# boqian-li/GarmentDreamer

Hardware: AMD Instinct MI355X
Metric: SDS iters/sec (rasterize+UNet+bwd), 100k Gaussians ×8 views @512², 1/2/4/8 GPU (higher is better)
Workload: dtype bf16

## Files before the change

garmentdreamer_amd/csrc/nn_conv3x3.hip:

```cpp
#include <hip/hip_runtime.h>
#include <stdlib.h>
#include <stdint.h>
#include <stdio.h>

#include <mutex>
#include <vector>

#include "../../include/gd_nn.h"
#include "nn_device.h"
#include "nn_host.h"

#ifndef GD_CONV_ABLATE
#define GD_CONV_ABLATE 0
#endif

namespace {

using namespace gdnn;

#ifndef GD_PATCH_EPI
#define GD_PATCH_EPI 0
#endif
typedef __attribute__((ext_vector_type(4))) float f32x4;

// ... 241 lines not shown

__device__ __forceinline__ float silu_fast(float z) { return z * __builtin_amdgcn_rcpf(1.0f + __expf(-z)); }

__device__ __forceinline__ float row16_sum(float v)
{
    v += __builtin_bit_cast(float, __builtin_amdgcn_update_dpp(0, __builtin_bit_cast(int, v), 0xB1, 0xf, 0xf, false));
    v += __builtin_bit_cast(float, __builtin_amdgcn_update_dpp(0, __builtin_bit_cast(int, v), 0x4E, 0xf, 0xf, false));
    v += __builtin_bit_cast(float, __builtin_amdgcn_update_dpp(0, __builtin_bit_cast(int, v), 0x141, 0xf, 0xf, false));
    v += __builtin_bit_cast(float, __builtin_amdgcn_update_dpp(0, __builtin_bit_cast(int, v), 0x140, 0xf, 0xf, false));
    return v;
}

__device__ __forceinline__ void stat_accumulate(float2& st, uint2 o)
{
    const float r0 = __uint_as_float(o.x << 16), r1 = __uint_as_float(o.x & 0xffff0000u);
    const float r2 = __uint_as_float(o.y << 16), r3 = __uint_as_float(o.y & 0xffff0000u);
    st.x += (r0 + r1) + (r2 + r3);
    st.y += fmaf(r0, r0, fmaf(r1, r1, fmaf(r2, r2, r3 * r3)));
}

__device__ __forceinline__ void patch_col(int fn, int& rr, int& fx)
{
    if (fn < 4) { rr = 0; fx = fn; }
    else if (fn < 12) { rr = 1; fx = fn - 4; }
    else if (fn < 16) { rr = 0; fx = fn - 8; }
    else if (fn < 20) { rr = 1; fx = fn - 8; }
    else if (fn < 28) { rr = 0; fx = fn - 12; }
    else { rr = 1; fx = fn - 16; }
}

constexpr int kTrRow = 80;
constexpr int kTrWave = 64 * kTrRow;

template <int BN, int WN, int FA, int FB>
__device__ __forceinline__ void patch_epilogue(f32x16 (&acc)[FA][FB], char* tr, int nimg, int tyi, int txi, int n0, int wc,
                                               int wp, int lane, int H, int W, int Cout, const uint16_t* __restrict__ bias,
                                               int bias_img_stride, const uint16_t* __restrict__ residual,
                                               uint16_t* __restrict__ out, float* __restrict__ stat_part, int tpi,
                                               int tiles_x)
{
    const int fk = lane >> 5, fn = lane & 31;
    int rr, fx;
    patch_col(fn, rr, fx);
    bool ok[FB];
    size_t opix[FB];
#pragma unroll
    for (int b = 0; b < FB; b++) {
        const int oy = tyi * 16 + 4 * wp + 2 * b + rr, ox = txi * 16 + fx;
        ok[b] = oy < H && ox < W;
        opix[b] = ((size_t)nimg * H + oy) * W + ox;
    }
    const uint16_t* bias_n = bias ? bias + (size_t)nimg * bias_img_stride : nullptr;
    const int stat_rows = tpi * 8;
    const int stat_row = (tyi * tiles_x + txi) * 8 + wp * 2 + ((lane >> 4) & 1);
    const bool wide = GD_PATCH_EPI != 2 && tr != nullptr && (Cout & 7) == 0;
#pragma unroll
    for (int a = 0; a < FA; a++) {
#pragma unroll
        for (int q = 0; q < 4; q++) {
            const int co = n0 + wc * (BN / WN) + a * 32 + 8 * q + 4 * fk;
            const bool cok = co < Cout;
            float bv[4] = {0.f, 0.f, 0.f, 0.f};
            if (bias_n && cok) {
                const uint2 bb = *(const uint2*)(bias_n + co);
                bv[0] = bf2f((uint16_t)(bb.x & 0xffff)); bv[1] = bf2f((uint16_t)(bb.x >> 16));
                bv[2] = bf2f((uint16_t)(bb.y & 0xffff)); bv[3] = bf2f((uint16_t)(bb.y >> 16));
            }
            float2 st = make_float2(0.f, 0.f);
#pragma unroll
            for (int b = 0; b < FB; b++) {
                if (!ok[b] || !cok) continue;
                float v[4];
#pragma unroll
                for (int e = 0; e < 4; e++) v[e] = acc[a][b][4 * q + e] + bv[e];
                if (residual) {
                    const uint2 rv = *(const uint2*)(residual + opix[b] * Cout + co);
                    v[0] += bf2f((uint16_t)(rv.x & 0xffff)); v[1] += bf2f((uint16_t)(rv.x >> 16));
                    v[2] += bf2f((uint16_t)(rv.y & 0xffff)); v[3] += bf2f((uint16_t)(rv.y >> 16));
                }
                uint2 o;
                o.x = pack_bf16(v[0], v[1]);
                o.y = pack_bf16(v[2], v[3]);
                if (wide) *(uint2*)(tr + (b * 32 + fn) * kTrRow + 16 * q + 8 * fk) = o;
                else if (GD_PATCH_EPI != 1 || H < 0) *(uint2*)(out + opix[b] * Cout + co) = o;
                if (stat_part) stat_accumulate(st, o);
            }
            if (stat_part) {
                const float sx = row16_sum(st.x), sy = row16_sum(st.y);
                if ((lane & 15) == 0 && cok)
                    *(float2*)(stat_part + (((size_t)nimg * (Cout >> 2) + (co >> 2)) * stat_rows + stat_row) * 2) =
                        make_float2(sx, sy);
            }
        }
        if (wide) {
            __builtin_amdgcn_wave_barrier();
#pragma unroll
            for (int i = 0; i < FB * 2; i++) {
                const int pr = (lane >> 2) + 16 * i, ch = lane & 3;
                int rr2, fx2;
                patch_col(pr & 31, rr2, fx2);
                const int oy = tyi * 16 + 4 * wp + 2 * (pr >> 5) + rr2, ox = txi * 16 + fx2;
                const int co8 = n0 + wc * (BN / WN) + a * 32 + 8 * ch;
                if (oy < H && ox < W && co8 < Cout) {
                    const uint4 v = *(const uint4*)(tr + pr * kTrRow + ch * 16);
                    if (GD_PATCH_EPI != 1 || H < 0) *(uint4*)(out + (((size_t)nimg * H + oy) * W + ox) * Cout + co8) = v;
                }
            }
            __builtin_amdgcn_wave_barrier();
        }
    }
}

template <int BN, int WN, int WM, bool GN>
__global__ __launch_bounds__(64 * WN * WM) void conv3x3_gn_patch_kernel(
    const uint16_t* __restrict__ in, const uint16_t* __restrict__ wt, const uint16_t* __restrict__ bias,
    int bias_img_stride, const uint16_t* __restrict__ residual, uint16_t* __restrict__ out, int Nimg, int H, int W,
    int Cin, int Cout, const float* __restrict__ mean_rstd, const uint16_t* __restrict__ gamma,
    const uint16_t* __restrict__ beta, int G, int apply_silu, int tiles_n, int tiles_x, int tiles_y, int nwg,
    float* __restrict__ stat_part)
{
    constexpr int BM = 256;
    constexpr int THREADS = 64 * WN * WM;
    constexpr int NB = BN * 8 / THREADS;
    constexpr int NA = (kPatchPix * 8 + THREADS - 1) / THREADS;
    constexpr int FA = BN / WN / 32, FB = BM / WM / 32;
    static_assert(FB == 2 && THREADS % 8 == 0, "wave pixel block = 4 patch rows x 16");
    constexpr int kAStage = (kPatchPix + 4) * BK * 2;
    constexpr int kBStage = BN * BK * 2;
    extern __shared__ __attribute__((aligned(16))) char smem[];
    char* sA = smem;
    char* sB = smem + 2 * kAStage;

    const int tid = threadIdx.x, lane = tid & 63;
    const int wave = __builtin_amdgcn_readfirstlane(tid >> 6);
    int bid = blockIdx.x;
    if ((nwg & 7) == 0) bid = (bid & 7) * (nwg >> 3) + (bid >> 3);
    const int tn = bid % tiles_n, tm = bid / tiles_n;
    const int tpi = tiles_x * tiles_y;
    const int nimg = tm / tpi, trem = tm - nimg * tpi;
// ... 133 lines not shown
                    if (tap == 0) loadA(c + 1);
                    else if (tap == 1) storeA((c + 1) & 1, c + 1);
                } else if (tap == 0) {
                    issueA((c + 1) & 1, c + 1);
                }
            }
            const char* pb = sB + bufB * kBStage;
            const int tapoff = (tap / 3) * kPatch + (tap % 3);
            uint32_t p_rd[FB], p_sw[FB];
#pragma unroll
            for (int b = 0; b < FB; b++) {
                const int p = p_base[b] + tapoff;
                p_rd[b] = (uint32_t)p * 128u;
                p_sw[b] = (uint32_t)((p >> 1) & 7);
            }
#pragma unroll
            for (int kk = 0; kk < 4; kk++) {
                bf16x8_t wf[FA], pf[FB];
#pragma unroll
                for (int a = 0; a < FA; a++) wf[a] = *(const bf16x8_t*)(pb + (w_rd[a] ^ (uint32_t)(kk << 5)));
#pragma unroll
                for (int b = 0; b < FB; b++)
                    pf[b] = *(const bf16x8_t*)(pa + p_rd[b] + ((((uint32_t)(2 * kk + fk)) ^ p_sw[b]) << 4));
#pragma unroll
                for (int a = 0; a < FA; a++)
#pragma unroll
                    for (int b = 0; b < FB; b++)
                        acc[a][b] = __builtin_amdgcn_mfma_f32_32x32x16_bf16(wf[a], pf[b], acc[a][b], 0, 0, 0);
            }
        }
    }

    if (GD_PATCH_EPI != 2) __syncthreads();
    patch_epilogue<BN, WN, FA, FB>(acc, sA + ((kc - 1) & 1) * kAStage + wave * kTrWave, nimg, tyi, txi, n0, wc, wp, lane, H, W,
                                   Cout, bias, bias_img_stride, residual, out, stat_part, tpi, tiles_x);
}

template <int BN, int WN, int WM, bool GN>
__global__ __launch_bounds__(64 * WN * WM) void conv3x3_patch_stream_kernel(
    const uint16_t* __restrict__ in, const uint16_t* __restrict__ wt, const uint16_t* __restrict__ bias,
    int bias_img_stride, const uint16_t* __restrict__ residual, uint16_t* __restrict__ out, int Nimg, int H, int W,
    int Cin, int Cout, const float* __restrict__ mean_rstd, const uint16_t* __restrict__ gamma,
    const uint16_t* __restrict__ beta, int G, int apply_silu, int tiles_n, int tiles_x, int tiles_y, int nwg,
    float* __restrict__ stat_part)
{
    constexpr int BM = 256;
    constexpr int THREADS = 64 * WN * WM;
    constexpr int NB = BN * 8 / THREADS;
    constexpr int NA = (kPatchPix * 8 + THREADS - 1) / THREADS;
    constexpr int FA = BN / WN / 32, FB = BM / WM / 32;
    static_assert(FB == 2 && THREADS % 8 == 0, "wave pixel block = 4 patch rows x 16");
    constexpr int kAStage = (kPatchPix + 4) * BK * 2;
    constexpr int kBStage = BN * BK * 2;
    extern __shared__ __attribute__((aligned(16))) char smem[];
    char* sA = smem;
    char* sB = smem + 2 * kAStage;

    const int tid = threadIdx.x, lane = tid & 63;
    const int wave = __builtin_amdgcn_readfirstlane(tid >> 6);
    const int tpi = tiles_x * tiles_y;
    const bool remap = (nwg & 7) == 0 && (GN || (gridDim.x & 7) == 0);
    struct Tile { int nimg, tyi, txi, n0; };
    auto decode = [&](int vb) {
        int bid = vb;
        if (remap) bid = (vb & 7) * (nwg >> 3) + (vb >> 3);
        const int tn = bid % tiles_n, tm = bid / tiles_n;
        Tile t;
        t.nimg = tm / tpi;
// ... 162 lines not shown
                        if (tap == 0) loadA(nc);
                        else if (tap == 1) storeA(st, nc);
                    } else if (tap == 0) {
                        issueA(st, nc);
                    }
                }
                const char* pb = sB + bufB * kBStage;
                const int tapoff = (tap / 3) * kPatch + (tap % 3);
                uint32_t p_rd[FB], p_sw[FB];
#pragma unroll
                for (int b = 0; b < FB; b++) {
                    const int p = p_base[b] + tapoff;
                    p_rd[b] = (uint32_t)p * 128u;
                    p_sw[b] = (uint32_t)((p >> 1) & 7);
                }
#pragma unroll
                for (int kk = 0; kk < 4; kk++) {
                    bf16x8_t wf[FA], pf[FB];
#pragma unroll
                    for (int a = 0; a < FA; a++) wf[a] = *(const bf16x8_t*)(pb + (w_rd[a] ^ (uint32_t)(kk << 5)));
#pragma unroll
                    for (int b = 0; b < FB; b++)
                        pf[b] = *(const bf16x8_t*)(pa + p_rd[b] + ((((uint32_t)(2 * kk + fk)) ^ p_sw[b]) << 4));
#pragma unroll
                    for (int a = 0; a < FA; a++)
#pragma unroll
                        for (int b = 0; b < FB; b++)
                            acc[a][b] = __builtin_amdgcn_mfma_f32_32x32x16_bf16(wf[a], pf[b], acc[a][b], 0, 0, 0);
                }
            }
        }

        if (GD_PATCH_EPI != 2) __syncthreads();
        patch_epilogue<BN, WN, FA, FB>(acc, sA + ((ga - 1) & 1) * kAStage + wave * kTrWave, cur.nimg, cur.tyi, cur.txi, cur.n0,
                                       wc, wp, lane, H, W, Cout, bias, bias_img_stride, residual, out, stat_part, tpi,
                                       tiles_x);
        if (!has_next) break;
        cur = nxt;
        vb = vnext;
#pragma unroll
        for (int a = 0; a < FA; a++)
#pragma unroll
            for (int b = 0; b < FB; b++)
#pragma unroll
                for (int k = 0; k < 16; k++) acc[a][b][k] = 0.f;
    }
}

#include "nn_conv_wino.h"
#include "nn_conv_wide.h"
#include "nn_conv_first_dgrad.h"
#ifdef GD_NN_EXPERIMENTAL_STREAM
#include "nn_conv_stream.h"
#endif
#ifdef GD_NN_EXPERIMENTAL_REGW
#include "nn_conv_regw.h"
#endif

template <int BM_T>
__global__ __launch_bounds__(256) void conv_splitk_reduce_kernel(const float* __restrict__ partial, int S, int nwg,
                                                                 int tiles_n, int64_t M, int Cout, int HWg, int Wg, int Hout,
                                                                 int Wout, int osy, int osx, int ooy, int oox,
                                                                 const uint16_t* __restrict__ bias, int bias_img_stride,
                                                                 const uint16_t* __restrict__ residual,
                                                                 uint16_t* __restrict__ out)
{
    constexpr int kQuads = 128 * BM_T / 4, kBlocks = kQuads / 256;
    const int tile = blockIdx.x / kBlocks;
    const int r = ((blockIdx.x % kBlocks) << 8) | threadIdx.x;
    const int lane = r & 63, q = (r >> 6) & 3, a = (r >> 8) & 1, b = (r >> 9) & 1, wave = r >> 10;
    const int tn = tile % tiles_n, tm = tile / tiles_n;
    const int64_t m = (int64_t)tm * BM_T + (wave >> 1) * 64 + b * 32 + (lane & 31);
    const int co = tn * 128 + (wave & 1) * 64 + a * 32 + 8 * q + 4 * (lane >> 5);
    if (m >= M || co >= Cout) return;
    float4 v = make_float4(0.f, 0.f, 0.f, 0.f);
    const float4* p = (const float4*)partial + (size_t)tile * kQuads + r;
    for (int sidx = 0; sidx < S; sidx++) {
        const float4 t = p[(size_t)sidx * nwg * kQuads];
        v.x += t.x; v.y += t.y; v.z += t.z; v.w += t.w;
    }
    const size_t nimg = (size_t)(m / HWg);
    const int rem = (int)(m - (int64_t)nimg * HWg);
    const int ga = rem / Wg, gb = rem - ga * Wg;
    const size_t o = ((nimg * Hout + (size_t)(ga * osy + ooy)) * Wout + (size_t)(gb * osx + oox)) * Cout + co;
    if (bias) {
        const uint2 bb = *(const uint2*)(bias + nimg * (size_t)bias_img_stride + co);
        v.x += bf2f((uint16_t)(bb.x & 0xffff)); v.y += bf2f((uint16_t)(bb.x >> 16));
        v.z += bf2f((uint16_t)(bb.y & 0xffff)); v.w += bf2f((uint16_t)(bb.y >> 16));
    }
    if (residual) {
        const uint2 rr = *(const uint2*)(residual + o);
        v.x += bf2f((uint16_t)(rr.x & 0xffff)); v.y += bf2f((uint16_t)(rr.x >> 16));
        v.z += bf2f((uint16_t)(rr.y & 0xffff)); v.w += bf2f((uint16_t)(rr.y >> 16));
    }
    uint2 ov;
    ov.x = pack_bf16(v.x, v.y);
    ov.y = pack_bf16(v.z, v.w);
    *(uint2*)(out + o) = ov;
}

template <int CIN>
__global__ __launch_bounds__(256) void conv3x3_first_kernel(const uint16_t* __restrict__ in,
                                                            const uint16_t* __restrict__ wt,
                                                            const uint16_t* __restrict__ bias,
                                                            uint16_t* __restrict__ out, int Nimg, int H, int W, int Cout)
{
    constexpr int PX = 4;
    extern __shared__ __attribute__((aligned(16))) float s_w[];
    const int K = 9 * CIN;
    for (int i = threadIdx.x; i < K * Cout; i += 256) {
        const int k = i / Cout, co = i - k * Cout;
        s_w[i] = bf2f(wt[(size_t)co * K + k]);
    }
    __syncthreads();
    const int octs = Cout >> 3;
    const int oct = threadIdx.x % octs, grp = threadIdx.x / octs;
    const int gpb = 256 / octs;
    const int gx = (W + PX - 1) / PX;
    const int64_t total = (int64_t)Nimg * H * gx;
    if (grp >= gpb) return;
    for (int64_t g = (int64_t)blockIdx.x * gpb + grp; g < total; g += (int64_t)gridDim.x * gpb) {
    const int n = (int)((uint32_t)g / (uint32_t)(H * gx));
    const int rem = (int)((uint32_t)g - (uint32_t)n * (uint32_t)(H * gx));
    const int y = rem / gx, x0 = (rem - y * gx) * PX;

    float acc[PX][8];
    {
// ... 238 lines not shown
        if (b) g_cprof.pool.push_back(b);
    }
    void close_s1(int64_t M, int Cin, int Cout, bool residual)
    {
        close(2.0 * (double)M * Cout * 9.0 * Cin,
              2.0 * ((double)M * Cin + 9.0 * Cin * Cout + (double)M * Cout + (residual ? (double)M * Cout : 0.0)));
    }
};

struct TiledArgs {
    void* stream;
    const void* x;
    const float* mean_rstd;
    const void *gamma, *beta;
    int groups, silu;
    const void *w, *bias;
    int bias_img_stride;
    const void* residual;
    void* y;
    int N, H, W, Cin, Cout;
    float* stat_part;
};
constexpr int kCuLds = 160 * 1024;
static bool gn_table_fits(int lds, int Cin) { return lds + gn_table_bytes(Cin) <= kCuLds; }
template <auto Kern>
int launch_tiled(const TiledArgs& a, int lds, int tile_w, int bn, bool persistent)
{
    const int dev = current_device();
    if (dev < 0) return dev;
    if (a.mean_rstd) {
        if (!gn_table_fits(lds, a.Cin)) return fail(GD_NN_ERR_INVALID_ARG, "GroupNorm scale / shift table of Cin channels does not fit the LDS");
        lds += gn_table_bytes(a.Cin);
    }
    if (const int r = reserve_lds<Kern>(dev, a.mean_rstd ? kCuLds : lds)) return r;
    hipStream_t s = (hipStream_t)a.stream;
    const int tiles_x = (a.W + tile_w - 1) / tile_w, tiles_y = (a.H + 15) / 16, tiles_n = (a.Cout + bn - 1) / bn;
    const int nwg = a.N * tiles_x * tiles_y * tiles_n;
    int grid = nwg;
    if (persistent && nwg > num_cus(dev)) grid = (nwg & 7) == 0 ? (num_cus(dev) & ~7) : num_cus(dev);
    ProfScope prof(s);
    hipLaunchKernelGGL(Kern, dim3(grid), dim3(512), lds, s, (const uint16_t*)a.x, (const uint16_t*)a.w,
                       (const uint16_t*)a.bias, a.bias_img_stride, (const uint16_t*)a.residual, (uint16_t*)a.y, a.N, a.H,
                       a.W, a.Cin, a.Cout, a.mean_rstd, (const uint16_t*)a.gamma, (const uint16_t*)a.beta, a.groups, a.silu,
                       tiles_n, tiles_x, tiles_y, nwg, a.stat_part);
    prof.close_s1((int64_t)a.N * a.H * a.W, a.Cin, a.Cout, a.residual != nullptr);
    return launch_status();
}

}

extern "C" {

const char* gd_nn_conv_last_error(void) { return g_err; }

static int pick_split(int64_t tiles, int steps, int target = 420)
{
    int s = (int)((target + tiles / 2) / tiles);
    const int cap = steps * 2 / 15 < 24 ? steps * 2 / 15 : 24;
    if (s > cap) s = cap;
    return s < 2 ? 1 : s;
}

static size_t split_ws_bytes(int split, int64_t M, int Cout)
{
    return (size_t)split * (size_t)((M + 255) / 256 * 2) * (size_t)((Cout + 127) / 128) * 16384u * sizeof(float);
}
// ... 718 lines not shown
```

garmentdreamer_amd/csrc/nn_conv_wide.h:

```cpp
#pragma once
#include "nn_device.h"

constexpr int kWideCK = 32;
constexpr int kWidePW = 34, kWidePix = 18 * kWidePW;
constexpr int kWidePStage = 2560 * 16;
constexpr int kWideWStage = 3 * 128 * kWideCK * 2;
constexpr int kWideLds = 2 * kWidePStage + 2 * kWideWStage;

__global__ __launch_bounds__(256) void conv3x3_wide_weights_kernel(const uint16_t* __restrict__ w, uint16_t* __restrict__ u,
                                                                   int Cout, int Cin)
{
    const int kc = Cin / kWideCK;
    const int tiles_n = (Cout + 127) / 128;
    const size_t total = (size_t)tiles_n * 3 * kc * 1536;
    for (size_t i = (size_t)blockIdx.x * blockDim.x + threadIdx.x; i < total; i += (size_t)gridDim.x * blockDim.x) {
        const int q = (int)(i % 1536);
        const size_t sl = i / 1536;
        const int c = (int)(sl % kc);
        const int ky = (int)((sl / kc) % 3);
        const int tn = (int)(sl / kc / 3);
        const int pc = q & 3, row = (q >> 2) & 127, kx = q >> 9;
        const int co = tn * 128 + row;
        const int ci0 = c * kWideCK + ((pc ^ ((row >> 2) & 3)) << 3);
        uint4 v = make_uint4(0u, 0u, 0u, 0u);
// ... 140 lines not shown
                    issueP((c + 1) & 1, c + 1);
                }
            }
            const char* pw = sW + bufW * kWideWStage;
#pragma unroll 1
            for (int kx = 0; kx < 3; kx++) {
                uint32_t p_rd[4], p_sw[4];
#pragma unroll
                for (int b = 0; b < 4; b++) {
                    const int p = p_base[b] + ky * kWidePW + kx;
                    p_rd[b] = (uint32_t)p * 64u;
                    p_sw[b] = (uint32_t)((p >> 2) & 3);
                }
#pragma unroll
                for (int kk = 0; kk < 2; kk++) {
                    const uint32_t ch = (uint32_t)(kk * 2 + fk);
                    bf16x8_t wf[2], pf[4];
#pragma unroll
                    for (int a = 0; a < 2; a++)
                        wf[a] = *(const bf16x8_t*)(pw + kx * (128 * 64) + a_rd[a] + ((ch ^ a_key) << 4));
#pragma unroll
                    for (int b = 0; b < 4; b++) pf[b] = *(const bf16x8_t*)(pa + p_rd[b] + ((ch ^ p_sw[b]) << 4));
#pragma unroll
                    for (int a = 0; a < 2; a++)
#pragma unroll
                        for (int b = 0; b < 4; b++)
                            acc[a][b] = __builtin_amdgcn_mfma_f32_32x32x16_bf16(wf[a], pf[b], acc[a][b], 0, 0, 0);
                }
            }
        }
    }

    __syncthreads();
    char* tr = smem + wave * kTrWave;
    const uint16_t* bias_n = bias ? bias + (size_t)nimg * bias_img_stride : nullptr;
    const int stat_rows = ((H + 15) / 16) * ((W + 15) / 16) * 8;
#pragma unroll
    for (int bh = 0; bh < 2; bh++) {
        bool ok[2];
        size_t opix[2];
#pragma unroll
        for (int j = 0; j < 2; j++) {
            const int oy = tyi * 16 + 4 * wr + 2 * j + rr, ox = txi * 32 + 16 * bh + fx;
            ok[j] = oy < H && ox < W;
            opix[j] = ((size_t)nimg * H + oy) * W + ox;
        }
        const int t16x = (W + 15) / 16, cx = 2 * txi + bh;
        const int stat_row = (tyi * t16x + cx) * 8 + wr * 2 + ((lane >> 4) & 1);
#pragma unroll
        for (int a = 0; a < 2; a++) {
#pragma unroll
            for (int q = 0; q < 4; q++) {
                const int co = n0 + wc * 64 + a * 32 + 8 * q + 4 * fk;
                const bool cok = co < Cout;
                float bv[4] = {0.f, 0.f, 0.f, 0.f};
                if (bias_n && cok) {
                    const uint2 bb = *(const uint2*)(bias_n + co);
                    bv[0] = bf2f((uint16_t)(bb.x & 0xffff)); bv[1] = bf2f((uint16_t)(bb.x >> 16));
                    bv[2] = bf2f((uint16_t)(bb.y & 0xffff)); bv[3] = bf2f((uint16_t)(bb.y >> 16));
                }
                float2 st = make_float2(0.f, 0.f);
#pragma unroll
                for (int j = 0; j < 2; j++) {
                    if (!ok[j] || !cok) continue;
                    const int b = 2 * bh + j;
                    float v[4];
#pragma unroll
                    for (int e = 0; e < 4; e++) v[e] = acc[a][b][4 * q + e] + bv[e];
                    if (residual) {
                        const uint2 rv = *(const uint2*)(residual + opix[j] * Cout + co);
                        v[0] += bf2f((uint16_t)(rv.x & 0xffff)); v[1] += bf2f((uint16_t)(rv.x >> 16));
                        v[2] += bf2f((uint16_t)(rv.y & 0xffff)); v[3] += bf2f((uint16_t)(rv.y >> 16));
                    }
                    uint2 o;
                    o.x = pack_bf16(v[0], v[1]);
                    o.y = pack_bf16(v[2], v[3]);
                    *(uint2*)(tr + (j * 32 + fn) * kTrRow + 16 * q + 8 * fk) = o;
                    if (stat_part) stat_accumulate(st, o);
                }
                if (stat_part) {
                    const float sx = row16_sum(st.x), sy = row16_sum(st.y);
                    if ((lane & 15) == 0 && cok && cx < t16x)
                        *(float2*)(stat_part + (((size_t)nimg * (Cout >> 2) + (co >> 2)) * stat_rows + stat_row) * 2) =
                            make_float2(sx, sy);
                }
            }
            __builtin_amdgcn_wave_barrier();
#pragma unroll
            for (int i = 0; i < 4; i++) {
                const int pr = (lane >> 2) + 16 * i, ch = lane & 3;
                int rr2, fx2;
                patch_col(pr & 31, rr2, fx2);
                const int oy = tyi * 16 + 4 * wr + 2 * (pr >> 5) + rr2, ox = txi * 32 + 16 * bh + fx2;
                const int co8 = n0 + wc * 64 + a * 32 + 8 * ch;
                if (oy < H && ox < W && co8 < Cout) {
                    const uint4 v = *(const uint4*)(tr + pr * kTrRow + ch * 16);
                    *(uint4*)(out + (((size_t)nimg * H + oy) * W + ox) * Cout + co8) = v;
                }
            }
            __builtin_amdgcn_wave_barrier();
        }
    }
}
```

garmentdreamer_amd/csrc/nn_conv_wino.h:

```cpp
#pragma once
#include "nn_device.h"

#ifndef GD_WINO_ABLATE
#define GD_WINO_ABLATE 0
#endif

constexpr int kWinoCK = 32;
constexpr int kWinoVStage = 4 * 18 * 8 * kWinoCK * 2;
constexpr int kWinoWStage = 4 * 128 * kWinoCK * 2;
constexpr int kWinoPBytes = 21 * 1024;
constexpr int kWinoLds = 2 * kWinoVStage + 2 * kWinoWStage + kWinoPBytes;

__device__ __forceinline__ uint16_t f2bf_finite(float f)
{
    uint32_t u = __float_as_uint(f);
    u += 0x7fffu + ((u >> 16) & 1u);
    return (uint16_t)(u >> 16);
}

__global__ __launch_bounds__(256) void conv3x3_wino_weights_kernel(const uint16_t* __restrict__ w,
                                                                   uint16_t* __restrict__ u, int Cout, int Cin)
{
    const int kc = Cin / kWinoCK;
    const int tiles_n = (Cout + 127) / 128;
// ... 214 lines not shown
#pragma unroll
                        for (int a = 0; a < 2; a++)
#pragma unroll
                            for (int b = 0; b < 2; b++) acc[p][a][b][0] += (float)wf[a][0] * (float)vf[b][1];
                    } else {
#pragma unroll
                        for (int a = 0; a < 2; a++)
#pragma unroll
                            for (int b = 0; b < 2; b++)
                                acc[p][a][b] = __builtin_amdgcn_mfma_f32_32x32x16_bf16(wf[a], vf[b], acc[p][a][b], 0, 0, 0);
                    }
                }
            }
        }
    }

    __syncthreads();
    if (GD_WINO_ABLATE != 5) {
        char* mine = smem + wave * 16384;
#pragma unroll
        for (int a = 0; a < 2; a++)
#pragma unroll
            for (int b = 0; b < 2; b++) {
#pragma unroll
                for (int q = 0; q < 4; q++) {
                    f32x4 sd;
#pragma unroll
                    for (int e = 0; e < 4; e++) sd[e] = pp ? acc[0][a][b][4 * q + e] : acc[1][a][b][4 * q + e];
                    *(f32x4*)(mine + ((a * 2 + b) * 4 + q) * 1024 + lane * 16) = sd;
                }
            }
    }
    __syncthreads();
    {
        const char* theirs = smem + (wave ^ 1) * 16384;
#pragma unroll
        for (int a = 0; a < 2; a++)
#pragma unroll
            for (int b = 0; b < 2; b++)
#pragma unroll
                for (int q = 0; q < 4; q++) {
                    const f32x4 rv = GD_WINO_ABLATE == 5 ? f32x4{0.f, 1.f, 2.f, 3.f}
                                                         : *(const f32x4*)(theirs + ((a * 2 + b) * 4 + q) * 1024 + lane * 16);
#pragma unroll
                    for (int e = 0; e < 4; e++) {
                        const float sm = acc[0][a][b][4 * q + e] + acc[1][a][b][4 * q + e];
                        acc[0][a][b][4 * q + e] = pp ? rv[e] - sm : sm + rv[e];
                    }
                }
    }
    __syncthreads();

    char* tr = smem + wave * kTrWave;
    bool ok[2];
    size_t opix[2];
#pragma unroll
    for (int b = 0; b < 2; b++) {
        const int oy = tyi * 16 + wq * 8 + b * 4 + (fn >> 3), ox = txi * 16 + 2 * (fn & 7) + pp;
        ok[b] = oy < H && ox < W;
        opix[b] = ((size_t)nimg * H + oy) * W + ox;
    }
    const uint16_t* bias_n = bias ? bias + (size_t)nimg * bias_img_stride : nullptr;
    const int stat_rows = tpi * 8;
    const int stat_row = (tyi * tiles_x + txi) * 8 + (pp * 2 + wq) * 2 + ((lane >> 4) & 1);
    const bool wide = (Cout & 7) == 0;
#pragma unroll
    for (int a = 0; a < 2; a++) {
#pragma unroll
        for (int q = 0; q < 4; q++) {
            const int co = n0 + wc * 64 + a * 32 + 8 * q + 4 * fk;
            const bool cok = co < Cout;
            float bv[4] = {0.f, 0.f, 0.f, 0.f};
            if (bias_n && cok) {
                const uint2 bb = *(const uint2*)(bias_n + co);
                bv[0] = bf2f((uint16_t)(bb.x & 0xffff)); bv[1] = bf2f((uint16_t)(bb.x >> 16));
                bv[2] = bf2f((uint16_t)(bb.y & 0xffff)); bv[3] = bf2f((uint16_t)(bb.y >> 16));
            }
            float2 st = make_float2(0.f, 0.f);
#pragma unroll
            for (int b = 0; b < 2; b++) {
                if (!ok[b] || !cok) continue;
                float v[4];
#pragma unroll
                for (int e = 0; e < 4; e++) v[e] = acc[0][a][b][4 * q + e] + bv[e];
                if (residual) {
                    const uint2 rv = *(const uint2*)(residual + opix[b] * Cout + co);
                    v[0] += bf2f((uint16_t)(rv.x & 0xffff)); v[1] += bf2f((uint16_t)(rv.x >> 16));
                    v[2] += bf2f((uint16_t)(rv.y & 0xffff)); v[3] += bf2f((uint16_t)(rv.y >> 16));
                }
                uint2 o;
                o.x = pack_bf16(v[0], v[1]);
                o.y = pack_bf16(v[2], v[3]);
                if (wide) *(uint2*)(tr + (b * 32 + fn) * kTrRow + 16 * q + 8 * fk) = o;
                else *(uint2*)(out + opix[b] * Cout + co) = o;
                if (stat_part) stat_accumulate(st, o);
            }
            if (stat_part) {
                const float sx = row16_sum(st.x), sy = row16_sum(st.y);
                if ((lane & 15) == 0 && cok)
                    *(float2*)(stat_part + (((size_t)nimg * (Cout >> 2) + (co >> 2)) * stat_rows + stat_row) * 2) =
                        make_float2(sx, sy);
            }
        }
        if (wide) {
            __builtin_amdgcn_wave_barrier();
#pragma unroll
            for (int i = 0; i < 4; i++) {
                const int pr = (lane >> 2) + 16 * i, ch = lane & 3;
                const int oy = tyi * 16 + wq * 8 + (pr >> 5) * 4 + ((pr & 31) >> 3), ox = txi * 16 + 2 * (pr & 7) + pp;
                const int co8 = n0 + wc * 64 + a * 32 + 8 * ch;
                if (oy < H && ox < W && co8 < Cout) {
                    const uint4 v = *(const uint4*)(tr + pr * kTrRow + ch * 16);
                    if (GD_WINO_ABLATE != 6 || H < 0) *(uint4*)(out + (((size_t)nimg * H + oy) * W + ox) * Cout + co8) = v;
                }
            }
            __builtin_amdgcn_wave_barrier();
        }
    }
}
```

garmentdreamer_amd/csrc/nn_device.h:

```cpp
#pragma once
#include <hip/hip_runtime.h>
#include <stdint.h>

namespace gdnn {

typedef __attribute__((ext_vector_type(8))) short bf16x8_t;
typedef __attribute__((ext_vector_type(16))) float f32x16;
typedef __attribute__((ext_vector_type(2))) float f32x2_t;
typedef __attribute__((ext_vector_type(2))) __bf16 bf16x2_t;
using f2 = f32x2_t;
using bf2_t = bf16x2_t;

struct alignas(16) bf16x8 {
    uint16_t v[8];
};
struct alignas(16) u32x4 { uint32_t w[4]; };

__device__ __forceinline__ float bf2f(uint16_t b) { return __uint_as_float(((uint32_t)b) << 16); }
__device__ __forceinline__ uint16_t f2bf(float f)
{
    uint32_t u = __float_as_uint(f);
    if ((u & 0x7fffffffu) > 0x7f800000u) return (uint16_t)((u >> 16) | 0x40);
    u += 0x7fffu + ((u >> 16) & 1u);
    return (uint16_t)(u >> 16);
}

__device__ __forceinline__ float lo16(uint32_t u) { return __uint_as_float(u << 16); }
__device__ __forceinline__ float hi16(uint32_t u) { return __uint_as_float(u & 0xffff0000u); }
__device__ __forceinline__ f2 unpack2(uint32_t w) { return f2{lo16(w), hi16(w)}; }
__device__ __forceinline__ uint32_t pack2(f2 v) { return __builtin_bit_cast(uint32_t, __builtin_convertvector(v, bf2_t)); }
__device__ __forceinline__ uint32_t pack_bf16(float lo, float hi) { return pack2(f2{lo, hi}); }
__device__ __forceinline__ f2 round_bf16(f2 v) { return unpack2(pack2(v)); }

__device__ __forceinline__ __amdgpu_buffer_rsrc_t buffer_rsrc(const void* p, uint32_t bytes)
{
    return __builtin_amdgcn_make_buffer_rsrc((void*)p, 0, (int)bytes, 0x00020000);
}

constexpr uint32_t kOOB = 0x80000000u;

__device__ __forceinline__ void bload_lds16(__amdgpu_buffer_rsrc_t rsrc, uint32_t voff, uint32_t soff, char* lds_wave_base)
{
    __builtin_amdgcn_raw_ptr_buffer_load_lds(rsrc, (__attribute__((address_space(3))) void*)lds_wave_base, 16, voff, soff,
                                             0, 0);
}

__device__ __forceinline__ int swz(int row, int j)
{
    return (row >> 1) * 256 + (((((row & 1) << 3) | j) ^ ((row >> 1) & 15)) << 4);
}

constexpr int gn_table_bytes(int Cin) { return 8 * Cin; }

__device__ __forceinline__ void gn_scale_shift(float gm, float bt, float mean, float rstd, float& sc, float& sh)
{
    sc = gm * rstd;
    sh = __builtin_fmaf(-mean, sc, bt);
}

__device__ __forceinline__ void gn_table_fill(uint32_t tab_off, int tid, int nthreads, int Cin, int G, int nimg,
                                              const float* __restrict__ mean_rstd, const uint16_t* __restrict__ gamma,
                                              const uint16_t* __restrict__ beta)
{
    const int cg = Cin / G;
    for (int ch = tid; ch < Cin; ch += nthreads) {
        const float2 mr = *(const float2*)(mean_rstd + ((size_t)nimg * G + ch / cg) * 2);
        float sc, sh;
        gn_scale_shift(bf2f(gamma[ch]), bf2f(beta[ch]), mr.x, mr.y, sc, sh);
        const uint32_t a = tab_off + (uint32_t)(((ch >> 3) * 16 + (ch & 7)) * 4);
        asm volatile("ds_write_b32 %0, %1\n\tds_write_b32 %0, %2 offset:32" ::"v"(a), "v"(sc), "v"(sh) : "memory");
    }
}

__device__ __forceinline__ void gn_table_sync()
{
    asm volatile("s_waitcnt lgkmcnt(0)" ::: "memory");
    __builtin_amdgcn_s_barrier();
}

__device__ __forceinline__ void gn_table_read(uint32_t tab_off, int octet, float (&sc)[8], float (&sh)[8])
{
    typedef __attribute__((ext_vector_type(4))) float f32x4;
// ... 12 lines not shown
```

Measured before the change: 23.03.

## Prefetch epilogue bias/residual via buffer loads and use OOB-masked buffer stores

Conv epilogues (patch, stream, wide, winograd) now preload bias and residual operands through raw buffer loads with out-of-bounds offsets in place of branches. Residuals are double-buffered one round ahead of use so global latency overlaps the pack/store work. Output stores become buffer stores with 32-bit offsets. Waves whose channel slice lies past Cout exit early, and the split-K reduce kernel issues its bias/residual loads before the partial-sum loop. This raises register pressure and caps one output image at 2 GiB, which the host now checks.

```diff
diff --git a/garmentdreamer_amd/csrc/nn_conv3x3.hip b/garmentdreamer_amd/csrc/nn_conv3x3.hip
--- a/garmentdreamer_amd/csrc/nn_conv3x3.hip
+++ b/garmentdreamer_amd/csrc/nn_conv3x3.hip
@@ -297,58 +297,87 @@
 constexpr int kTrRow = 80;
 constexpr int kTrWave = 64 * kTrRow;
 
-template <int BN, int WN, int FA, int FB>
+template <int BN, int WN, int FA, int FB, bool DB, int QB = 4>
 __device__ __forceinline__ void patch_epilogue(f32x16 (&acc)[FA][FB], char* tr, int nimg, int tyi, int txi, int n0, int wc,
                                                int wp, int lane, int H, int W, int Cout, const uint16_t* __restrict__ bias,
                                                int bias_img_stride, const uint16_t* __restrict__ residual,
                                                uint16_t* __restrict__ out, float* __restrict__ stat_part, int tpi,
                                                int tiles_x)
 {
+    if (n0 + wc * (BN / WN) >= Cout) return;
     const int fk = lane >> 5, fn = lane & 31;
     int rr, fx;
     patch_col(fn, rr, fx);
     bool ok[FB];
-    size_t opix[FB];
+    uint32_t rpix[FB];
 #pragma unroll
     for (int b = 0; b < FB; b++) {
         const int oy = tyi * 16 + 4 * wp + 2 * b + rr, ox = txi * 16 + fx;
         ok[b] = oy < H && ox < W;
-        opix[b] = ((size_t)nimg * H + oy) * W + ox;
-    }
-    const uint16_t* bias_n = bias ? bias + (size_t)nimg * bias_img_stride : nullptr;
+        rpix[b] = (uint32_t)(oy * W + ox) * (uint32_t)Cout * 2u;
+    }
+    const __amdgpu_buffer_rsrc_t rs_out = buffer_rsrc(out + (size_t)nimg * H * W * Cout, (uint32_t)(H * W) * (uint32_t)Cout * 2u);
+    uint32_t spix[FB * 2];
+#pragma unroll
+    for (int i = 0; i < FB * 2; i++) {
+        const int pr = (lane >> 2) + 16 * i;
+        int rr2, fx2;
+        patch_col(pr & 31, rr2, fx2);
+        const int oy = tyi * 16 + 4 * wp + 2 * (pr >> 5) + rr2, ox = txi * 16 + fx2;
+        spix[i] = oy < H && ox < W ? (uint32_t)(oy * W + ox) * (uint32_t)Cout * 2u : kOOB;
+    }
+    const EpiOperands eo(bias, bias_img_stride, residual, nimg, (uint32_t)(H * W) * (uint32_t)Cout, Cout);
+    const int cbase = n0 + wc * (BN / WN) + 4 * fk;
+    constexpr int NQ = DB ? 4 : QB;
+    uint2 bb[DB ? FA : 1][NQ] = {}, rv[DB ? 2 : 1][NQ][FB] = {};
+    auto load_batch = [&](int a, int q0) {
+        if (!DB) {
+#pragma unroll
+            for (int i = 0; i < NQ; i++) bb[0][i] = eo.load_bias(cbase + a * 32 + 8 * (q0 + i));
+        }
+        if (!DB || residual) {
+#pragma unroll
+            for (int i = 0; i < NQ; i++) {
+                const int co = cbase + a * 32 + 8 * (q0 + i);
+#pragma unroll
+                for (int b = 0; b < FB; b++)
+                    rv[DB ? a & 1 : 0][i][b] = eo.load_residual(ok[b] && co < Cout ? rpix[b] + (uint32_t)co * 2u : kOOB);
+            }
+        }
+    };
+    if (DB && bias) {
+#pragma unroll
+        for (int a = 0; a < FA; a++)
+#pragma unroll
+            for (int q = 0; q < 4; q++) bb[a][q] = eo.load_bias(cbase + a * 32 + 8 * q);
+    }
+    load_batch(0, 0);
     const int stat_rows = tpi * 8;
     const int stat_row = (tyi * tiles_x + txi) * 8 + wp * 2 + ((lane >> 4) & 1);
     const bool wide = GD_PATCH_EPI != 2 && tr != nullptr && (Cout & 7) == 0;
 #pragma unroll
     for (int a = 0; a < FA; a++) {
+        if (DB && a + 1 < FA) load_batch(a + 1, 0);
 #pragma unroll
         for (int q = 0; q < 4; q++) {
-            const int co = n0 + wc * (BN / WN) + a * 32 + 8 * q + 4 * fk;
+            const int co = cbase + a * 32 + 8 * q;
             const bool cok = co < Cout;
-            float bv[4] = {0.f, 0.f, 0.f, 0.f};
-            if (bias_n && cok) {
-                const uint2 bb = *(const uint2*)(bias_n + co);
-                bv[0] = bf2f((uint16_t)(bb.x & 0xffff)); bv[1] = bf2f((uint16_t)(bb.x >> 16));
-                bv[2] = bf2f((uint16_t)(bb.y & 0xffff)); bv[3] = bf2f((uint16_t)(bb.y >> 16));
-            }
             float2 st = make_float2(0.f, 0.f);
 #pragma unroll
             for (int b = 0; b < FB; b++) {
-                if (!ok[b] || !cok) continue;
+                const bool m = ok[b] && cok;
                 float v[4];
 #pragma unroll
-                for (int e = 0; e < 4; e++) v[e] = acc[a][b][4 * q + e] + bv[e];
-                if (residual) {
-                    const uint2 rv = *(const uint2*)(residual + opix[b] * Cout + co);
-                    v[0] += bf2f((uint16_t)(rv.x & 0xffff)); v[1] += bf2f((uint16_t)(rv.x >> 16));
-                    v[2] += bf2f((uint16_t)(rv.y & 0xffff)); v[3] += bf2f((uint16_t)(rv.y >> 16));
-                }
+                for (int e = 0; e < 4; e++) v[e] = acc[a][b][4 * q + e];
+                epi_add(v, bb[DB ? a : 0][q % NQ]);
+                epi_add(v, rv[DB ? a & 1 : 0][q % NQ][b]);
                 uint2 o;
                 o.x = pack_bf16(v[0], v[1]);
                 o.y = pack_bf16(v[2], v[3]);
                 if (wide) *(uint2*)(tr + (b * 32 + fn) * kTrRow + 16 * q + 8 * fk) = o;
-                else if (GD_PATCH_EPI != 1 || H < 0) *(uint2*)(out + opix[b] * Cout + co) = o;
-                if (stat_part) stat_accumulate(st, o);
+                else if (GD_PATCH_EPI != 1 || H < 0)
+                    __builtin_amdgcn_raw_buffer_store_b64(u32x2_t{o.x, o.y}, rs_out, (int)(m ? rpix[b] + (uint32_t)co * 2u : kOOB), 0, 0);
+                if (stat_part) stat_accumulate(st, m ? o : make_uint2(0u, 0u));
             }
             if (stat_part) {
                 const float sx = row16_sum(st.x), sy = row16_sum(st.y);
@@ -356,20 +385,20 @@
                     *(float2*)(stat_part + (((size_t)nimg * (Cout >> 2) + (co >> 2)) * stat_rows + stat_row) * 2) =
                         make_float2(sx, sy);
             }
+            if (!DB && (q + 1) % NQ == 0) {
+                if (q + 1 < 4) load_batch(a, q + 1);
+                else if (a + 1 < FA) load_batch(a + 1, 0);
+            }
         }
         if (wide) {
             __builtin_amdgcn_wave_barrier();
+            const int co8 = n0 + wc * (BN / WN) + a * 32 + 8 * (lane & 3);
 #pragma unroll
             for (int i = 0; i < FB * 2; i++) {
                 const int pr = (lane >> 2) + 16 * i, ch = lane & 3;
-                int rr2, fx2;
-                patch_col(pr & 31, rr2, fx2);
-                const int oy = tyi * 16 + 4 * wp + 2 * (pr >> 5) + rr2, ox = txi * 16 + fx2;
-                const int co8 = n0 + wc * (BN / WN) + a * 32 + 8 * ch;
-                if (oy < H && ox < W && co8 < Cout) {
-                    const uint4 v = *(const uint4*)(tr + pr * kTrRow + ch * 16);
-                    if (GD_PATCH_EPI != 1 || H < 0) *(uint4*)(out + (((size_t)nimg * H + oy) * W + ox) * Cout + co8) = v;
-                }
+                const u32x4_t v = *(const u32x4_t*)(tr + pr * kTrRow + ch * 16);
+                if (GD_PATCH_EPI != 1 || H < 0)
+                    __builtin_amdgcn_raw_buffer_store_b128(v, rs_out, (int)(co8 < Cout ? spix[i] + (uint32_t)co8 * 2u : kOOB), 0, 0);
             }
             __builtin_amdgcn_wave_barrier();
         }
@@ -569,8 +598,8 @@
     }
 
     if (GD_PATCH_EPI != 2) __syncthreads();
-    patch_epilogue<BN, WN, FA, FB>(acc, sA + ((kc - 1) & 1) * kAStage + wave * kTrWave, nimg, tyi, txi, n0, wc, wp, lane, H, W,
-                                   Cout, bias, bias_img_stride, residual, out, stat_part, tpi, tiles_x);
+    patch_epilogue<BN, WN, FA, FB, true>(acc, sA + ((kc - 1) & 1) * kAStage + wave * kTrWave, nimg, tyi, txi, n0, wc, wp,
+                                         lane, H, W, Cout, bias, bias_img_stride, residual, out, stat_part, tpi, tiles_x);
 }
 
 template <int BN, int WN, int WM, bool GN>
@@ -799,9 +828,10 @@
         }
 
         if (GD_PATCH_EPI != 2) __syncthreads();
-        patch_epilogue<BN, WN, FA, FB>(acc, sA + ((ga - 1) & 1) * kAStage + wave * kTrWave, cur.nimg, cur.tyi, cur.txi, cur.n0,
-                                       wc, wp, lane, H, W, Cout, bias, bias_img_stride, residual, out, stat_part, tpi,
-                                       tiles_x);
+        __builtin_amdgcn_sched_barrier(0);
+        patch_epilogue<BN, WN, FA, FB, BN == 128, 2>(acc, sA + ((ga - 1) & 1) * kAStage + wave * kTrWave, cur.nimg, cur.tyi,
+                                                  cur.txi, cur.n0, wc, wp, lane, H, W, Cout, bias, bias_img_stride, residual,
+                                                  out, stat_part, tpi, tiles_x);
         if (!has_next) break;
         cur = nxt;
         vb = vnext;
@@ -840,26 +870,21 @@
     const int64_t m = (int64_t)tm * BM_T + (wave >> 1) * 64 + b * 32 + (lane & 31);
     const int co = tn * 128 + (wave & 1) * 64 + a * 32 + 8 * q + 4 * (lane >> 5);
     if (m >= M || co >= Cout) return;
+    const size_t nimg = (size_t)(m / HWg);
+    const int rem = (int)(m - (int64_t)nimg * HWg);
+    const int ga = rem / Wg, gb = rem - ga * Wg;
+    const size_t o = ((nimg * Hout + (size_t)(ga * osy + ooy)) * Wout + (size_t)(gb * osx + oox)) * Cout + co;
+    uint2 bb = make_uint2(0u, 0u), rr = make_uint2(0u, 0u);
+    if (bias) bb = *(const uint2*)(bias + nimg * (size_t)bias_img_stride + co);
+    if (residual) rr = *(const uint2*)(residual + o);
     float4 v = make_float4(0.f, 0.f, 0.f, 0.f);
     const float4* p = (const float4*)partial + (size_t)tile * kQuads + r;
     for (int sidx = 0; sidx < S; sidx++) {
         const float4 t = p[(size_t)sidx * nwg * kQuads];
         v.x += t.x; v.y += t.y; v.z += t.z; v.w += t.w;
     }
-    const size_t nimg = (size_t)(m / HWg);
-    const int rem = (int)(m - (int64_t)nimg * HWg);
-    const int ga = rem / Wg, gb = rem - ga * Wg;
-    const size_t o = ((nimg * Hout + (size_t)(ga * osy + ooy)) * Wout + (size_t)(gb * osx + oox)) * Cout + co;
-    if (bias) {
-        const uint2 bb = *(const uint2*)(bias + nimg * (size_t)bias_img_stride + co);
-        v.x += bf2f((uint16_t)(bb.x & 0xffff)); v.y += bf2f((uint16_t)(bb.x >> 16));
-        v.z += bf2f((uint16_t)(bb.y & 0xffff)); v.w += bf2f((uint16_t)(bb.y >> 16));
-    }
-    if (residual) {
-        const uint2 rr = *(const uint2*)(residual + o);
-        v.x += bf2f((uint16_t)(rr.x & 0xffff)); v.y += bf2f((uint16_t)(rr.x >> 16));
-        v.z += bf2f((uint16_t)(rr.y & 0xffff)); v.w += bf2f((uint16_t)(rr.y >> 16));
-    }
+    v.x += lo16(bb.x); v.y += hi16(bb.x); v.z += lo16(bb.y); v.w += hi16(bb.y);
+    v.x += lo16(rr.x); v.y += hi16(rr.x); v.z += lo16(rr.y); v.w += hi16(rr.y);
     uint2 ov;
     ov.x = pack_bf16(v.x, v.y);
     ov.y = pack_bf16(v.z, v.w);
@@ -1164,6 +1189,8 @@
         if (!gn_table_fits(lds, a.Cin)) return fail(GD_NN_ERR_INVALID_ARG, "GroupNorm scale / shift table of Cin channels does not fit the LDS");
         lds += gn_table_bytes(a.Cin);
     }
+    if ((double)a.H * a.W * a.Cout * 2.0 >= 2147483648.0)
+        return fail(GD_NN_ERR_INVALID_ARG, "conv3x3: one image of the output must be < 2 GiB (32-bit buffer offsets)");
     if (const int r = reserve_lds<Kern>(dev, a.mean_rstd ? kCuLds : lds)) return r;
     hipStream_t s = (hipStream_t)a.stream;
     const int tiles_x = (a.W + tile_w - 1) / tile_w, tiles_y = (a.H + 15) / 16, tiles_n = (a.Cout + bn - 1) / bn;
diff --git a/garmentdreamer_amd/csrc/nn_conv_wide.h b/garmentdreamer_amd/csrc/nn_conv_wide.h
--- a/garmentdreamer_amd/csrc/nn_conv_wide.h
+++ b/garmentdreamer_amd/csrc/nn_conv_wide.h
@@ -196,51 +196,67 @@
     }
 
     __syncthreads();
+    if (n0 + wc * 64 >= Cout) return;
     char* tr = smem + wave * kTrWave;
-    const uint16_t* bias_n = bias ? bias + (size_t)nimg * bias_img_stride : nullptr;
     const int stat_rows = ((H + 15) / 16) * ((W + 15) / 16) * 8;
-#pragma unroll
-    for (int bh = 0; bh < 2; bh++) {
-        bool ok[2];
-        size_t opix[2];
+    const EpiOperands eo(bias, bias_img_stride, residual, nimg, (uint32_t)(H * W) * (uint32_t)Cout, Cout);
+    const __amdgpu_buffer_rsrc_t rs_out = buffer_rsrc(out + (size_t)nimg * H * W * Cout, (uint32_t)(H * W) * (uint32_t)Cout * 2u);
+    const int cbase = n0 + wc * 64 + 4 * fk;
+    bool ok[2][2];
+    uint32_t rpix[2][2];
+#pragma unroll
+    for (int bh = 0; bh < 2; bh++)
 #pragma unroll
         for (int j = 0; j < 2; j++) {
             const int oy = tyi * 16 + 4 * wr + 2 * j + rr, ox = txi * 32 + 16 * bh + fx;
-            ok[j] = oy < H && ox < W;
-            opix[j] = ((size_t)nimg * H + oy) * W + ox;
-        }
+            ok[bh][j] = oy < H && ox < W;
+            rpix[bh][j] = (uint32_t)(oy * W + ox) * (uint32_t)Cout * 2u;
+        }
+    uint2 bb[2][4] = {}, rv[2][4][2] = {};
+    auto load_round = [&](int r) {
+        const int bh = r >> 1, a = r & 1;
+        if (!residual) return;
+#pragma unroll
+        for (int q = 0; q < 4; q++) {
+            const int co = cbase + a * 32 + 8 * q;
+#pragma unroll
+            for (int j = 0; j < 2; j++)
+                rv[r & 1][q][j] = eo.load_residual(ok[bh][j] && co < Cout ? rpix[bh][j] + (uint32_t)co * 2u : kOOB);
+        }
+    };
+    if (bias) {
+#pragma unroll
+        for (int a = 0; a < 2; a++)
+#pragma unroll
+            for (int q = 0; q < 4; q++) bb[a][q] = eo.load_bias(cbase + a * 32 + 8 * q);
+    }
+    load_round(0);
+#pragma unroll
+    for (int bh = 0; bh < 2; bh++) {
         const int t16x = (W + 15) / 16, cx = 2 * txi + bh;
         const int stat_row = (tyi * t16x + cx) * 8 + wr * 2 + ((lane >> 4) & 1);
 #pragma unroll
         for (int a = 0; a < 2; a++) {
+            const int r = 2 * bh + a;
+            if (r + 1 < 4) load_round(r + 1);
 #pragma unroll
             for (int q = 0; q < 4; q++) {
-                const int co = n0 + wc * 64 + a * 32 + 8 * q + 4 * fk;
+                const int co = cbase + a * 32 + 8 * q;
                 const bool cok = co < Cout;
-                float bv[4] = {0.f, 0.f, 0.f, 0.f};
-                if (bias_n && cok) {
-                    const uint2 bb = *(const uint2*)(bias_n + co);
-                    bv[0] = bf2f((uint16_t)(bb.x & 0xffff)); bv[1] = bf2f((uint16_t)(bb.x >> 16));
-                    bv[2] = bf2f((uint16_t)(bb.y & 0xffff)); bv[3] = bf2f((uint16_t)(bb.y >> 16));
-                }
                 float2 st = make_float2(0.f, 0.f);
 #pragma unroll
                 for (int j = 0; j < 2; j++) {
-                    if (!ok[j] || !cok) continue;
                     const int b = 2 * bh + j;
                     float v[4];
 #pragma unroll
-                    for (int e = 0; e < 4; e++) v[e] = acc[a][b][4 * q + e] + bv[e];
-                    if (residual) {
-                        const uint2 rv = *(const uint2*)(residual + opix[j] * Cout + co);
-                        v[0] += bf2f((uint16_t)(rv.x & 0xffff)); v[1] += bf2f((uint16_t)(rv.x >> 16));
-                        v[2] += bf2f((uint16_t)(rv.y & 0xffff)); v[3] += bf2f((uint16_t)(rv.y >> 16));
-                    }
+                    for (int e = 0; e < 4; e++) v[e] = acc[a][b][4 * q + e];
+                    epi_add(v, bb[a][q]);
+                    epi_add(v, rv[r & 1][q][j]);
                     uint2 o;
                     o.x = pack_bf16(v[0], v[1]);
                     o.y = pack_bf16(v[2], v[3]);
                     *(uint2*)(tr + (j * 32 + fn) * kTrRow + 16 * q + 8 * fk) = o;
-                    if (stat_part) stat_accumulate(st, o);
+                    if (stat_part) stat_accumulate(st, ok[bh][j] && cok ? o : make_uint2(0u, 0u));
                 }
                 if (stat_part) {
                     const float sx = row16_sum(st.x), sy = row16_sum(st.y);
@@ -257,10 +273,9 @@
                 patch_col(pr & 31, rr2, fx2);
                 const int oy = tyi * 16 + 4 * wr + 2 * (pr >> 5) + rr2, ox = txi * 32 + 16 * bh + fx2;
                 const int co8 = n0 + wc * 64 + a * 32 + 8 * ch;
-                if (oy < H && ox < W && co8 < Cout) {
-                    const uint4 v = *(const uint4*)(tr + pr * kTrRow + ch * 16);
-                    *(uint4*)(out + (((size_t)nimg * H + oy) * W + ox) * Cout + co8) = v;
-                }
+                const u32x4_t v = *(const u32x4_t*)(tr + pr * kTrRow + ch * 16);
+                __builtin_amdgcn_raw_buffer_store_b128(
+                    v, rs_out, (int)(oy < H && ox < W && co8 < Cout ? (uint32_t)((oy * W + ox) * Cout + co8) * 2u : kOOB), 0, 0);
             }
             __builtin_amdgcn_wave_barrier();
         }
diff --git a/garmentdreamer_amd/csrc/nn_conv_wino.h b/garmentdreamer_amd/csrc/nn_conv_wino.h
--- a/garmentdreamer_amd/csrc/nn_conv_wino.h
+++ b/garmentdreamer_amd/csrc/nn_conv_wino.h
@@ -270,6 +270,35 @@
             }
     }
     __syncthreads();
+    bool ok[2];
+    uint32_t rpix[2];
+#pragma unroll
+    for (int b = 0; b < 2; b++) {
+        const int oy = tyi * 16 + wq * 8 + b * 4 + (fn >> 3), ox = txi * 16 + 2 * (fn & 7) + pp;
+        ok[b] = oy < H && ox < W;
+        rpix[b] = (uint32_t)(oy * W + ox) * (uint32_t)Cout * 2u;
+    }
+    const __amdgpu_buffer_rsrc_t rs_out = buffer_rsrc(out + (size_t)nimg * H * W * Cout, (uint32_t)(H * W) * (uint32_t)Cout * 2u);
+    const EpiOperands eo(bias, bias_img_stride, residual, nimg, (uint32_t)(H * W) * (uint32_t)Cout, Cout);
+    const int cbase = n0 + wc * 64 + 4 * fk;
+    uint2 bb[2][4] = {}, rsd[2][4][2] = {};
+    auto load_round = [&](int a) {
+        if (!residual) return;
+#pragma unroll
+        for (int q = 0; q < 4; q++) {
+            const int co = cbase + a * 32 + 8 * q;
+#pragma unroll
+            for (int b = 0; b < 2; b++)
+                rsd[a][q][b] = eo.load_residual(ok[b] && co < Cout ? rpix[b] + (uint32_t)co * 2u : kOOB);
+        }
+    };
+    if (bias) {
+#pragma unroll
+        for (int a = 0; a < 2; a++)
+#pragma unroll
+            for (int q = 0; q < 4; q++) bb[a][q] = eo.load_bias(cbase + a * 32 + 8 * q);
+    }
+    load_round(0);
     {
         const char* theirs = smem + (wave ^ 1) * 16384;
 #pragma unroll
@@ -287,51 +316,40 @@
                     }
                 }
     }
-    __syncthreads();
+#pragma unroll
+    for (int a = 0; a < 2; a++)
+#pragma unroll
+        for (int b = 0; b < 2; b++) asm volatile("" : "+v"(acc[0][a][b]));
+    __syncthreads();
+    if (n0 + wc * 64 >= Cout) return;
 
     char* tr = smem + wave * kTrWave;
-    bool ok[2];
-    size_t opix[2];
-#pragma unroll
-    for (int b = 0; b < 2; b++) {
-        const int oy = tyi * 16 + wq * 8 + b * 4 + (fn >> 3), ox = txi * 16 + 2 * (fn & 7) + pp;
-        ok[b] = oy < H && ox < W;
-        opix[b] = ((size_t)nimg * H + oy) * W + ox;
-    }
-    const uint16_t* bias_n = bias ? bias + (size_t)nimg * bias_img_stride : nullptr;
     const int stat_rows = tpi * 8;
     const int stat_row = (tyi * tiles_x + txi) * 8 + (pp * 2 + wq) * 2 + ((lane >> 4) & 1);
     const bool wide = (Cout & 7) == 0;
 #pragma unroll
     for (int a = 0; a < 2; a++) {
+        if (a + 1 < 2) load_round(a + 1);
 #pragma unroll
         for (int q = 0; q < 4; q++) {
-            const int co = n0 + wc * 64 + a * 32 + 8 * q + 4 * fk;
+            const int co = cbase + a * 32 + 8 * q;
             const bool cok = co < Cout;
-            float bv[4] = {0.f, 0.f, 0.f, 0.f};
-            if (bias_n && cok) {
-                const uint2 bb = *(const uint2*)(bias_n + co);
-                bv[0] = bf2f((uint16_t)(bb.x & 0xffff)); bv[1] = bf2f((uint16_t)(bb.x >> 16));
-                bv[2] = bf2f((uint16_t)(bb.y & 0xffff)); bv[3] = bf2f((uint16_t)(bb.y >> 16));
-            }
             float2 st = make_float2(0.f, 0.f);
 #pragma unroll
             for (int b = 0; b < 2; b++) {
-                if (!ok[b] || !cok) continue;
+                const bool m = ok[b] && cok;
                 float v[4];
 #pragma unroll
-                for (int e = 0; e < 4; e++) v[e] = acc[0][a][b][4 * q + e] + bv[e];
-                if (residual) {
-                    const uint2 rv = *(const uint2*)(residual + opix[b] * Cout + co);
-                    v[0] += bf2f((uint16_t)(rv.x & 0xffff)); v[1] += bf2f((uint16_t)(rv.x >> 16));
-                    v[2] += bf2f((uint16_t)(rv.y & 0xffff)); v[3] += bf2f((uint16_t)(rv.y >> 16));
-                }
+                for (int e = 0; e < 4; e++) v[e] = acc[0][a][b][4 * q + e];
+                epi_add(v, bb[a][q]);
+                epi_add(v, rsd[a][q][b]);
                 uint2 o;
                 o.x = pack_bf16(v[0], v[1]);
                 o.y = pack_bf16(v[2], v[3]);
                 if (wide) *(uint2*)(tr + (b * 32 + fn) * kTrRow + 16 * q + 8 * fk) = o;
-                else *(uint2*)(out + opix[b] * Cout + co) = o;
-                if (stat_part) stat_accumulate(st, o);
+                else
+                    __builtin_amdgcn_raw_buffer_store_b64(u32x2_t{o.x, o.y}, rs_out, (int)(m ? rpix[b] + (uint32_t)co * 2u : kOOB), 0, 0);
+                if (stat_part) stat_accumulate(st, m ? o : make_uint2(0u, 0u));
             }
             if (stat_part) {
                 const float sx = row16_sum(st.x), sy = row16_sum(st.y);
@@ -347,10 +365,10 @@
                 const int pr = (lane >> 2) + 16 * i, ch = lane & 3;
                 const int oy = tyi * 16 + wq * 8 + (pr >> 5) * 4 + ((pr & 31) >> 3), ox = txi * 16 + 2 * (pr & 7) + pp;
                 const int co8 = n0 + wc * 64 + a * 32 + 8 * ch;
-                if (oy < H && ox < W && co8 < Cout) {
-                    const uint4 v = *(const uint4*)(tr + pr * kTrRow + ch * 16);
-                    if (GD_WINO_ABLATE != 6 || H < 0) *(uint4*)(out + (((size_t)nimg * H + oy) * W + ox) * Cout + co8) = v;
-                }
+                const u32x4_t v = *(const u32x4_t*)(tr + pr * kTrRow + ch * 16);
+                if (GD_WINO_ABLATE != 6 || H < 0)
+                    __builtin_amdgcn_raw_buffer_store_b128(
+                        v, rs_out, (int)(oy < H && ox < W && co8 < Cout ? (uint32_t)((oy * W + ox) * Cout + co8) * 2u : kOOB), 0, 0);
             }
             __builtin_amdgcn_wave_barrier();
         }
diff --git a/garmentdreamer_amd/csrc/nn_device.h b/garmentdreamer_amd/csrc/nn_device.h
--- a/garmentdreamer_amd/csrc/nn_device.h
+++ b/garmentdreamer_amd/csrc/nn_device.h
@@ -8,6 +8,8 @@
 typedef __attribute__((ext_vector_type(16))) float f32x16;
 typedef __attribute__((ext_vector_type(2))) float f32x2_t;
 typedef __attribute__((ext_vector_type(2))) __bf16 bf16x2_t;
+typedef __attribute__((ext_vector_type(2))) uint32_t u32x2_t;
+typedef __attribute__((ext_vector_type(4))) uint32_t u32x4_t;
 using f2 = f32x2_t;
 using bf2_t = bf16x2_t;
 
@@ -48,6 +50,28 @@
 __device__ __forceinline__ int swz(int row, int j)
 {
     return (row >> 1) * 256 + (((((row & 1) << 3) | j) ^ ((row >> 1) & 15)) << 4);
+}
+
+struct EpiOperands {
+    __amdgpu_buffer_rsrc_t bias, res;
+    __device__ __forceinline__ EpiOperands(const uint16_t* b, int bias_img_stride, const uint16_t* r, int nimg,
+                                           uint32_t img_elems, int Cout)
+        : bias(buffer_rsrc(b ? b + (size_t)nimg * bias_img_stride : nullptr, b ? (uint32_t)Cout * 2u : 0u)),
+          res(buffer_rsrc(r ? r + (size_t)nimg * img_elems : nullptr, r ? img_elems * 2u : 0u))
+    {
+    }
+    __device__ __forceinline__ uint2 load(__amdgpu_buffer_rsrc_t rs, uint32_t voff) const
+    {
+        return __builtin_bit_cast(uint2, __builtin_amdgcn_raw_buffer_load_b64(rs, (int)voff, 0, 0));
+    }
+    __device__ __forceinline__ uint2 load_bias(int co) const { return load(bias, (uint32_t)co * 2u); }
+    __device__ __forceinline__ uint2 load_residual(uint32_t voff) const { return load(res, voff); }
+};
+
+__device__ __forceinline__ void epi_add(float (&v)[4], uint2 w)
+{
+    v[0] += lo16(w.x); v[1] += hi16(w.x);
+    v[2] += lo16(w.y); v[3] += hi16(w.y);
 }
 
 constexpr int gn_table_bytes(int Cin) { return 8 * Cin; }
```

Measured after the change: 23.24, median of 6. About the same (+0.9%).
